# google-research/multinerf

Measured on AMD Instinct MI355X. Metric: train_rays_per_sec, higher is better.
Workload: dtype bf16 MFMA inputs / fp32 accumulate, fp32 everywhere else

## Files before the change

### include/mnerf.h

```cpp
#ifndef MNERF_H_
#define MNERF_H_

#include <stdint.h>

#ifdef __cplusplus
extern "C" {
#endif

typedef enum {
  MNR_OK = 0,
  MNR_ERR_INVALID_ARGUMENT = -1,
  MNR_ERR_HIP = -2,
  MNR_ERR_UNSUPPORTED = -3
} mnr_status;

const char* mnr_last_error(void);
int mnr_abi_version(void);
int mnr_device_info(int device, int* cu_count, int* lds_bytes_per_cu, char* arch_name, int arch_name_len);

typedef enum { MNR_RAYDIST_IDENTITY = 0, MNR_RAYDIST_RECIPROCAL = 1, MNR_RAYDIST_PIECEWISE = 2,
               MNR_RAYDIST_LOG = 3, MNR_RAYDIST_EXP = 4, MNR_RAYDIST_SQRT = 5, MNR_RAYDIST_SQUARE = 6 } mnr_raydist;

typedef struct {
  int n_prev;
// ... 201 lines not shown
  float density_noise_std;
  int has_rgb;
  int rgb_act;
  float rgb_premultiplier, rgb_bias, rgb_padding;
  int bg_mode;
  float bg_value;
} mnr_composite_cfg;

int mnr_composite_fwd(const mnr_composite_cfg* cfg, int64_t B, const float* raw_density,
                      const float* density_noise, const float* raw_rgb, const float* tdist,
                      const float* dirs, const float* bg, const float* exposure_scale,
                      float* density, float* rgb, float* weights, float* rgb_out, float* acc,
                      void* stream);

int mnr_composite_bwd(const mnr_composite_cfg* cfg, int64_t B, const float* raw_density,
                      const float* density_noise, const float* raw_rgb, const float* tdist,
                      const float* dirs, const float* bg, const float* exposure_scale,
                      const float* weights, const float* g_rgb_out, const float* g_weights,
                      float* g_raw_density, uint16_t* g_raw_density_bf16, int ld_bf16,
                      float* g_raw_rgb, float* g_exposure_scale , void* stream);

typedef struct {
  mnr_composite_cfg cfg;
  int64_t B, B_valid;
  const float* raw_density; const float* density_noise; const float* raw_rgb; const float* tdist; const float* dirs;
  const float* bg; const float* exposure_scale; const float* weights;
  const float* g_rgb_out;
  const float* g_weights;
  float* g_raw_density; uint16_t* g_raw_density_bf16; int ld_bf16; float* g_raw_rgb; float* g_exposure_scale;
  int data_loss_type; float charb_padding; float data_loss_mult;
  const float* rgb_out; const float* gt; const float* lossmult; int lm_c; const float* denom; float* data_stats;
  int wloss_mode; float wloss_mult; const float* sdist; int n_ref; const float* t_ref; const float* w_ref; float* wloss_stat;
  float* g_x;
} mnr_level_bwd_args;
int mnr_level_bwd(const mnr_level_bwd_args* args, void* stream);

typedef struct {
  int64_t B, B_valid; int n;
  const float* sdist; const float* near; const float* far; int raydist_fn;
  const float* g_x; const float* raw_density; const float* density_noise; float density_noise_std; float density_bias;
  int density_act; const float* dirs;
  const float* g_t0; const float* g_t1;
  float distortion_mult; const float* weights;
  const float* g_sdist_in;
  float* g_sdist;
} mnr_sdist_bwd_args;
int mnr_sdist_bwd(const mnr_sdist_bwd_args* args, void* stream);

int mnr_exposure_scale(int64_t B, const float* exposure_values, const int32_t* exposure_idx,
                       const float* offsets, float* out, void* stream);
int mnr_exposure_scale_bwd(int64_t B_valid, const float* exposure_values, const int32_t* exposure_idx,
                           const float* g_scale, float* g_offsets, void* stream);

int mnr_render_extras(int64_t B, int n, const float* weights, const float* tdist, const float* t_far,
                      float* out, void* stream);

typedef struct {
  int T; int lmax;
  const int32_t* m; const int32_t* l;
  const float* sigma;
  const float* mat;
} mnr_ide_tables;

#define MNR_REF_PRED_NORMALS    1
#define MNR_REF_DENSITY_NORMALS 2
#define MNR_REF_REFLECT         4
// ... 385 lines not shown
```

### include/mnerf_debug.h

```cpp
#ifndef MNERF_DEBUG_H_
#define MNERF_DEBUG_H_

#ifdef __cplusplus
extern "C" {
#endif

int mnr_debug_gemm_timeline(unsigned long long* device_buffer);
int mnr_gemm_nt_set_pipelined(int on);
int mnr_gemm_nt_set_persistent(int wgs_per_cu);
int mnr_gemm_nt_set_wres(int max_wgs);
int mnr_gemm_nt_panel_set_max_wgs(int n);

int mnr_mlp_chain_set_deferred(int on);

int mnr_mlp_chain_set_max_wgs(int n);

int mnr_debug_chain_timeline(unsigned long long* device_buffer);

int mnr_level_bwd_set_quad(int on);

#ifdef __cplusplus
}
#endif
#endif
```

### multinerf_amd/_lib.py

```python

import ctypes as C
import os
import re

HERE = os.path.dirname(os.path.abspath(__file__))
LIB_PATH = os.environ.get('MNR_LIB_PATH') or os.path.join(HERE, 'libmnerf_hip.so')
LIB_F32_PATH = os.path.join(HERE, 'libmnerf_hip_f32.so')
HEADER_PATH = os.path.join(os.path.dirname(HERE), 'include', 'mnerf.h')
F32_ABSENT = ('mnr_mlp_chain_fwd', 'mnr_mlp_chain_fwd_ipe', 'mnr_mlp_chain_bwd')


def describe():
  stamp = LIB_PATH + '.stamp'
  digest = None
  if os.path.exists(stamp):
    with open(stamp) as f:
      digest = f.read().strip()
  return {'path': os.path.relpath(LIB_PATH, os.path.dirname(HERE)), 'overridden': bool(os.environ.get('MNR_LIB_PATH')),
          'source_digest': digest, 'extra_hipcc_flags': os.environ.get('MNR_EXTRA_HIPCC_FLAGS', '')}

MNR_OK = 0
MNR_ERR_INVALID_ARGUMENT = -1

RAYDIST = {None: 0, 'identity': 0, 'reciprocal': 1, 'piecewise': 2, 'log': 3, 'exp': 4, 'sqrt': 5,
# ... 63 lines not shown
  _fields_ = [('cfg', IpeCfg), ('n', C.c_int), ('tdist', vp), ('origins', vp), ('directions', vp), ('radii', vp),
              ('basis', vp)]


class MlpChainBwdArgs(C.Structure):
  _fields_ = [('M', C.c_int64), ('W', C.c_int), ('depth', C.c_int),
              ('g_head', vp), ('w_head', vp),
              ('bits', vp * CHAIN_MAX_DEPTH), ('Bw', vp * CHAIN_MAX_DEPTH), ('ldb', C.c_int * CHAIN_MAX_DEPTH),
              ('dY', vp * CHAIN_MAX_DEPTH), ('dY_in', vp)]


class PackDesc(C.Structure):
  _fields_ = [('src_off', C.c_int64), ('rows_in', C.c_int), ('cols_out', C.c_int),
              ('dst_off', C.c_int64), ('ld', C.c_int), ('row0', C.c_int), ('col0', C.c_int),
              ('transpose', C.c_int)]


class CompositeCfg(C.Structure):
  _fields_ = [('n', C.c_int), ('opaque_background', C.c_int), ('density_act', C.c_int),
              ('density_bias', C.c_float), ('density_noise_std', C.c_float), ('has_rgb', C.c_int),
              ('rgb_act', C.c_int), ('rgb_premultiplier', C.c_float), ('rgb_bias', C.c_float),
              ('rgb_padding', C.c_float), ('bg_mode', C.c_int), ('bg_value', C.c_float)]


class LevelBwdArgs(C.Structure):
  _fields_ = [('cfg', CompositeCfg), ('B', C.c_int64), ('B_valid', C.c_int64),
              ('raw_density', vp), ('density_noise', vp), ('raw_rgb', vp), ('tdist', vp), ('dirs', vp),
              ('bg', vp), ('exposure_scale', vp), ('weights', vp), ('g_rgb_out', vp), ('g_weights', vp),
              ('g_raw_density', vp), ('g_raw_density_bf16', vp), ('ld_bf16', C.c_int), ('g_raw_rgb', vp),
              ('g_exposure_scale', vp),
              ('data_loss_type', C.c_int), ('charb_padding', C.c_float), ('data_loss_mult', C.c_float),
              ('rgb_out', vp), ('gt', vp), ('lossmult', vp), ('lm_c', C.c_int), ('denom', vp), ('data_stats', vp),
              ('wloss_mode', C.c_int), ('wloss_mult', C.c_float), ('sdist', vp), ('n_ref', C.c_int), ('t_ref', vp),
              ('w_ref', vp), ('wloss_stat', vp), ('g_x', vp)]


class SdistBwdArgs(C.Structure):
  _fields_ = [('B', C.c_int64), ('B_valid', C.c_int64), ('n', C.c_int),
              ('sdist', vp), ('near', vp), ('far', vp), ('raydist_fn', C.c_int),
              ('g_x', vp), ('raw_density', vp), ('density_noise', vp), ('density_noise_std', C.c_float),
              ('density_bias', C.c_float), ('density_act', C.c_int), ('dirs', vp),
              ('g_t0', vp), ('g_t1', vp), ('distortion_mult', C.c_float), ('weights', vp),
              ('g_sdist_in', vp), ('g_sdist', vp)]


class IdeTables(C.Structure):
  _fields_ = [('T', C.c_int), ('lmax', C.c_int), ('m', vp), ('l', vp), ('sigma', vp), ('mat', vp)]


class RobustArgs(C.Structure):
  _fields_ = [('B', C.c_int64), ('B_valid', C.c_int64),
              ('patch_size', C.c_int), ('inner_patch_size', C.c_int), ('filter_size', C.c_int), ('enable', C.c_int),
              ('smoothed_inlier_quantile', C.c_double), ('inner_patch_inlier_quantile', C.c_double),
              ('rgb', vp), ('gt', vp), ('lossmult', vp), ('lm_c', C.c_int), ('loss_threshold', vp), ('denom', vp),
              ('mask', vp), ('lossmult_out', vp), ('err', vp), ('stats', vp), ('mse', vp)]


SSIM_MAX_FILTER = 11
CC_FEATURES, CC_GRAM_OUT = 10, 65


class SsimArgs(C.Structure):
  _fields_ = [('H', C.c_int), ('W', C.c_int), ('C', C.c_int), ('crop', C.c_int), ('filter_size', C.c_int),
              ('filter_sigma', C.c_double), ('max_val', C.c_double), ('k1', C.c_double), ('k2', C.c_double),
              ('a', vp), ('b', vp), ('map', vp), ('partials', vp), ('out', vp)]


# ... 207 lines not shown
    'mnr_atlas_uvs': ([C.POINTER(AtlasArgs), vp, vp], i32),
    'mnr_raster_visibility': ([C.POINTER(RasterArgs), vp, vp, vp, vp], i32),
    'mnr_raster_shade': ([C.POINTER(RasterArgs), vp, vp, vp, vp, vp, vp, vp, vp], i32),
    'mnr_shtex_weights': ([vp, i64, vp, i64, vp, vp], i32),
    'mnr_shtex_fit': ([vp, vp, i64, i32, vp, vp, i64, C.c_double, vp, vp], i32),
    'mnr_shtex_shade': ([C.POINTER(ShtexShadeArgs), vp, vp], i32),
    'mnr_mesh_grid_count': ([C.POINTER(MeshDistArgs), vp, vp], i32),
    'mnr_mesh_grid_fill': ([C.POINTER(MeshDistArgs), vp, i64, vp, vp, vp], i32),
    'mnr_mesh_distance': ([C.POINTER(MeshDistArgs), vp, vp, i64, vp, vp, i64, f32, vp, vp, vp, vp], i32),
    'mnr_mesh_face_areas': ([vp, i64, vp, i64, vp, vp], i32),
    'mnr_mesh_sample': ([vp, i64, vp, i64, vp, i64, C.c_uint32, vp, vp, vp], i32),
    'mnr_mesh_closest': ([vp, i64, vp, i64, vp, vp, vp, i64, vp, vp, vp], i32),
    'mnr_mesh_face_normals': ([vp, i64, vp, i64, vp, vp], i32),
    'mnr_icp_sums_partials': ([i64], i32),
    'mnr_icp_sums': ([i64, vp, vp, vp, vp, C.POINTER(C.c_double), vp, vp, vp], i32),
    'mnr_crop_polygon': ([vp, i64, vp, i32, i32, C.c_double, C.c_double, vp, vp], i32),
    'mnr_mesh_raycast': ([C.POINTER(MeshDistArgs), vp, vp, i64, vp, vp, vp, i64, f32, f32, i32, vp, vp, vp, vp], i32),
    'mnr_raycast_shade': ([C.POINTER(RasterArgs), vp, vp, i64, vp, vp, vp], i32),
    'mnr_weight_decay': ([vp, i64, i64, f32, vp, vp, vp, vp], i32),
    'mnr_grad_sqnorm': ([vp, i64, i64, f32, vp, vp], i32),
    'mnr_clip_adam': ([C.POINTER(AdamCfg), i64, i64, vp, vp, vp, vp, vp, vp], i32),
}

_DEBUG_PROTOS = {
    'mnr_debug_gemm_timeline': ([vp], i32),
    'mnr_gemm_nt_set_persistent': ([i32], i32),
    'mnr_level_bwd_set_quad': ([i32], i32),
    'mnr_gemm_nt_set_pipelined': ([i32], i32),
    'mnr_gemm_nt_set_wres': ([i32], i32),
    'mnr_gemm_nt_panel_set_max_wgs': ([i32], i32),
    'mnr_debug_chain_timeline': ([vp], i32),
    'mnr_mlp_chain_set_deferred': ([i32], i32),
    'mnr_mlp_chain_set_max_wgs': ([i32], i32),
}

_lib = None


def header_symbols(path=None):
  with open(path or HEADER_PATH) as f:
    text = f.read()
  text = re.sub(r'/\*.*?\*/', '', text, flags=re.S)
  return sorted(set(re.findall(r'\b(mnr_[a-z0-9_]+)\s*\(', text)))


def _bind(path, absent=()):
  if not os.path.exists(path):
    raise RuntimeError(
        f'{path} is missing: the HIP extension has not been built. Run '
        '`python -m multinerf_amd.build` (needs hipcc, ROCm >= 7.0). There is no CPU fallback.')
  import torch
  lib = C.CDLL(path)
  lib.mnr_last_error.restype = C.c_char_p
  lib.mnr_last_error.argtypes = []
  for name, (argtypes, restype) in _PROTOS.items():
    if name in absent:
      continue
    fn = getattr(lib, name)
    fn.argtypes = argtypes
    fn.restype = restype
  return lib


_lib_f32 = None
_f32_depth = 0

# ... 54 lines not shown
```

### multinerf_amd/csrc/gemm.hip

```cpp
#include <stdio.h>
#include <stdlib.h>
#include <type_traits>

#include "common.h"

#ifdef MNR_DENSE_F32
#include "dense_f32.inc"
#else


#define NT_CPAD 16

template <int MI_, int NJ_, int WM_, int WN_, int EPI_BATCH_ = 0, int BIAS_LDS_ = 0, int PIPE_ = 0, int DBG_ = 0, int BK_ = 64, int STAGES_ = 2>
struct NtCfg {
  static constexpr int DBG = DBG_;
  static constexpr bool PIPE = PIPE_ != 0;
  static constexpr int EPI_BATCH = EPI_BATCH_;
  static constexpr int MI = MI_, NJ = NJ_, WM = WM_, WN = WN_, BK = BK_, STAGES = STAGES_;
  static constexpr int MINW = 1;
  static constexpr int BM = 32 * MI * WM, BN = 32 * NJ * WN;
  static constexpr int THREADS = 64 * WM * WN;
  static constexpr int ROWB = BK * 2;
  static constexpr int SLOTS = ROWB / 16;
  static constexpr int A_BYTES = BM * ROWB, B_BYTES = BN * ROWB;
// ... 540 lines not shown
  if (rl < row_lanes) {
    for (int64_t r = r0 + rl; r < r1; r += row_lanes) {
      const bf16x8 v = *(const bf16x8*)(X + r * ld + cg * 8);
#pragma unroll
      for (int e = 0; e < 8; ++e) s[e] += (float)v[e];
    }
  }
#pragma unroll
  for (int e = 0; e < 8; ++e) red[threadIdx.x * 8 + e] = s[e];
  __syncthreads();
  if (rl == 0) {
    for (int k = 1; k < row_lanes; ++k)
#pragma unroll
      for (int e = 0; e < 8; ++e) s[e] += red[(k * lanes_per_row + cg) * 8 + e];
#pragma unroll
    for (int e = 0; e < 8; ++e)
      if (cg * 8 + e < n_valid) unsafeAtomicAdd(out + cg * 8 + e, s[e]);
  }
}

extern "C" int mnr_colsum_bf16(const uint16_t* X, int ld, int64_t M, int n_valid, float* out, void* stream) {
  MNR_CHECK_ARG(X && out && M > 0 && n_valid > 0, "mnr_colsum_bf16: bad arguments");
  MNR_CHECK_ARG(ld % 8 == 0 && (n_valid + 7) / 8 <= 256 && ((n_valid + 7) / 8) * 8 <= ld,
                "mnr_colsum_bf16: need ld %% 8 == 0 and n_valid <= min(ld, 2048)");
  const int rows_per_block = 1024;
  const int grid = mnr_cdiv(M, rows_per_block);
  hipLaunchKernelGGL(colsum_kernel, dim3(grid), dim3(256), 0, (hipStream_t)stream, (const bf16*)X, ld, M,
                     n_valid, rows_per_block, out);
  MNR_CHECK_LAUNCH();
  return MNR_OK;
}


__global__ void pack_weights_kernel(const float* __restrict__ params, const mnr_pack_desc* __restrict__ descs,
                                    bf16* __restrict__ dst) {
  const mnr_pack_desc d = descs[blockIdx.y];
  const int total = d.rows_in * d.cols_out;
  for (int e = blockIdx.x * blockDim.x + threadIdx.x; e < total; e += gridDim.x * blockDim.x) {
    int r, c;
    if (d.transpose) {
      c = e / d.rows_in;
      r = e % d.rows_in;
    } else {
      r = e / d.cols_out;
      c = e % d.cols_out;
    }
    const float v = params[d.src_off + (int64_t)r * d.cols_out + c];
    const int64_t o = d.transpose ? d.dst_off + (int64_t)(d.row0 + c) * d.ld + d.col0 + r
                                  : d.dst_off + (int64_t)(d.row0 + r) * d.ld + d.col0 + c;
    dst[o] = (bf16)v;
  }
}

extern "C" int mnr_pack_weights_bf16(const float* params, const mnr_pack_desc* descs_device, int n_desc,
                                     int max_elems, uint16_t* dst, void* stream) {
  MNR_CHECK_ARG(params && descs_device && dst && n_desc > 0 && max_elems > 0, "mnr_pack_weights_bf16: bad arguments");
  int gx = mnr_cdiv(max_elems, 256);
  if (gx > 64) gx = 64;
  hipLaunchKernelGGL(pack_weights_kernel, dim3(gx, n_desc), dim3(256), 0, (hipStream_t)stream, params,
                     descs_device, (bf16*)dst);
  MNR_CHECK_LAUNCH();
  return MNR_OK;
}

__global__ void scatter_add_kernel(const float* __restrict__ src, int ld_src, int row0, int col0, int rows,
                                   int cols, float* __restrict__ dst, int ld_dst) {
  const int total = rows * cols;
  for (int e = blockIdx.x * blockDim.x + threadIdx.x; e < total; e += gridDim.x * blockDim.x) {
    const int k = e / cols, c = e % cols;
    dst[(int64_t)k * ld_dst + c] += src[(int64_t)(row0 + k) * ld_src + col0 + c];
  }
}

extern "C" int mnr_scatter_add_f32(const float* src, int ld_src, int row0, int col0, int rows, int cols,
                                   float* dst, int ld_dst, void* stream) {
  MNR_CHECK_ARG(src && dst && rows > 0 && cols > 0, "mnr_scatter_add_f32: bad arguments");
  int grid = mnr_cdiv((long long)rows * cols, 256);
  if (grid > 2048) grid = 2048;
  hipLaunchKernelGGL(scatter_add_kernel, dim3(grid), dim3(256), 0, (hipStream_t)stream, src, ld_src, row0,
                     col0, rows, cols, dst, ld_dst);
  MNR_CHECK_LAUNCH();
  return MNR_OK;
}

__global__ void cast_f32_bf16_kernel(const float* __restrict__ src, int ld_src, int64_t M, int n,
                                     bf16* __restrict__ dst, int ld_dst, int col0) {
  const int64_t total = M * n;
  for (int64_t e = (int64_t)blockIdx.x * blockDim.x + threadIdx.x; e < total; e += (int64_t)gridDim.x * blockDim.x) {
    const int64_t r = e / n;
    const int c = (int)(e % n);
    dst[r * ld_dst + col0 + c] = (bf16)src[r * ld_src + c];
// ... 299 lines not shown
```

### multinerf_amd/csrc/render.hip

```cpp
#include "common.h"
#include "ray_losses.h"

#define CP_THREADS 64

__device__ __forceinline__ float cp_act(int kind, float x) {
  switch (kind) {
    case MNR_ACT_SIGMOID: return mnr_sigmoid(x);
    case MNR_ACT_SAFE_EXP: return expf(fminf(x, 88.0f));
    case MNR_ACT_SOFTPLUS: return mnr_softplus(x);
    case MNR_ACT_EXP: return expf(x);
    case MNR_ACT_RELU: return fmaxf(x, 0.0f);
    default: return x;
  }
}

__device__ __forceinline__ float cp_act_grad(int kind, float x, float y) {
  switch (kind) {
    case MNR_ACT_SIGMOID: return y * (1.0f - y);
    case MNR_ACT_SAFE_EXP: return y;
    case MNR_ACT_SOFTPLUS: return mnr_sigmoid(x);
    case MNR_ACT_EXP: return y;
    case MNR_ACT_RELU: return x > 0.0f ? 1.0f : 0.0f;
    default: return 1.0f;
  }
// ... 440 lines not shown
        carry += Lanes<LPR>::suffix_total(inc);
        if (in) {
          float gx = ghat * l_tn[i] - after;
          if (c.opaque_background && i == n - 1) gx = 0.0f;
          l_den[i] = gx * l_dg[i];
          l_gh[i] = gx;
        }
      }
    }
    if (a.g_exposure_scale) {
#pragma unroll
      for (int ch = 0; ch < 3; ++ch) {
        const float g = Lanes<LPR>::sum(ges[ch]);
        if (live && q == 0) a.g_exposure_scale[ray * 3 + ch] += g;
      }
    }
  }
  if (a.data_loss_type >= 0 && a.data_stats) {
    s_mse = ls_wave_sum(s_mse);
    s_dloss = ls_wave_sum(s_dloss);
    if (threadIdx.x == 0) {
      const float denom = *a.denom;
      unsafeAtomicAdd(a.data_stats + 0, s_mse / denom);
      unsafeAtomicAdd(a.data_stats + 1, a.data_loss_mult * s_dloss / denom);
    }
  }
  if (a.wloss_mode != 0 && a.wloss_stat) {
    s_wloss = ls_wave_sum(s_wloss);
    const float norm = a.wloss_mode == 1 ? (float)a.B_valid * (float)a.n_ref : (float)a.B_valid;
    if (threadIdx.x == 0) unsafeAtomicAdd(a.wloss_stat, a.wloss_mult * s_wloss / norm);
  }
  __syncthreads();
  if (a.g_raw_density) cp_rows_out(lds, L.stride, L.den, a.g_raw_density + ray0 * n, rows, n);
  if (a.g_raw_density_bf16) {
    bf16* gb = (bf16*)a.g_raw_density_bf16;
    for (int e = threadIdx.x; e < rows * n; e += CP_THREADS) {
      const int rr = e / n, i = e - rr * n;
      gb[(ray0 * n + e) * (int64_t)a.ld_bf16] = (bf16)lds[rr * L.stride + L.den + i];
    }
  }
  if (c.has_rgb && a.g_raw_rgb) cp_rows_out(lds, L.stride, L.rgb, a.g_raw_rgb + ray0 * n * 3, rows, 3 * n);
  if (a.g_x) cp_rows_out(lds, L.stride, L.scr + 2 * n, a.g_x + ray0 * n, rows, n);
}

template <int LPR>
static void level_bwd_launch(const CpPlan& p, const mnr_level_bwd_args* a, void* stream) {
  static unsigned long long attr_set = 0;
  if (p.lds > 64 * 1024 && mnr_attr_needed(&attr_set))
    (void)hipFuncSetAttribute((const void*)level_bwd_kernel<LPR>, hipFuncAttributeMaxDynamicSharedMemorySize, 160 * 1024);
  hipLaunchKernelGGL(level_bwd_kernel<LPR>, dim3(mnr_cdiv(a->B, p.rays)), dim3(CP_THREADS), p.lds, (hipStream_t)stream, *a, p.rays);
}

extern "C" int mnr_level_bwd(const mnr_level_bwd_args* a, void* stream) {
  MNR_CHECK_ARG(a != nullptr, "mnr_level_bwd: null args");
  const mnr_composite_cfg* cfg = &a->cfg;
  MNR_CHECK_ARG(a->B > 0 && a->B_valid > 0 && a->B_valid <= a->B && a->raw_density && a->tdist && a->dirs && a->weights,
                "mnr_level_bwd: null argument");
  MNR_CHECK_ARG(cfg->n >= 1 && cfg->n <= 1024, "mnr_level_bwd: n out of range");
  MNR_CHECK_ARG(a->g_raw_density || a->g_raw_density_bf16, "mnr_level_bwd: no density-gradient output");
  MNR_CHECK_ARG(!cfg->has_rgb || a->raw_rgb, "mnr_level_bwd: has_rgb needs raw_rgb");
  MNR_CHECK_ARG(cfg->bg_mode == 0 || a->bg, "mnr_level_bwd: bg_mode 1 needs bg");
  MNR_CHECK_ARG(a->data_loss_type < 0 || (a->data_loss_type <= MNR_LOSS_RAWNERF && a->rgb_out && a->gt && a->lossmult &&
                                          a->denom && (a->lm_c == 1 || a->lm_c == 3)),
                "mnr_level_bwd: the fused data loss needs rgb_out, gt, lossmult [B,1|3] and denom");
  MNR_CHECK_ARG(a->wloss_mode >= 0 && a->wloss_mode <= 2, "mnr_level_bwd: wloss_mode must be 0, 1 or 2");
  MNR_CHECK_ARG(a->wloss_mode == 0 || a->sdist, "mnr_level_bwd: weight losses need this level's sdist");
  MNR_CHECK_ARG(a->wloss_mode != 1 || (a->n_ref >= 1 && a->n_ref <= 1024 && a->t_ref && a->w_ref),
                "mnr_level_bwd: the interlevel loss needs the final level's (t_ref, w_ref)");
  const CpPlan p = cp_plan(cfg->n, cfg->has_rgb, true, a->wloss_mode, a->n_ref, a->B);
  MNR_CHECK_ARG(p.lds <= 160 * 1024, "mnr_level_bwd: n=%d too long for LDS staging", cfg->n);
  (p.lpr == 4 ? level_bwd_launch<4> : level_bwd_launch<1>)(p, a, stream);
// ... 233 lines not shown
```

### multinerf_amd/csrc/resample.hip

```cpp
#include "common.h"

#pragma clang fp contract(off)

#define RS_THREADS 64

__device__ __forceinline__ float rs_s_to_t(int fn, float s, float near, float far) {
  float fn_near, fn_far;
  switch (fn) {
    case MNR_RAYDIST_RECIPROCAL: fn_near = 1.0f / near; fn_far = 1.0f / far; break;
    case MNR_RAYDIST_PIECEWISE:
      fn_near = near < 1.0f ? 0.5f * near : 1.0f - 0.5f / near;
      fn_far = far < 1.0f ? 0.5f * far : 1.0f - 0.5f / far;
      break;
    case MNR_RAYDIST_LOG: fn_near = logf(near); fn_far = logf(far); break;
    case MNR_RAYDIST_EXP: fn_near = expf(near); fn_far = expf(far); break;
    case MNR_RAYDIST_SQRT: fn_near = sqrtf(near); fn_far = sqrtf(far); break;
    case MNR_RAYDIST_SQUARE: fn_near = near * near; fn_far = far * far; break;
    default: fn_near = near; fn_far = far; break;
  }
  const float x = s * fn_far + (1.0f - s) * fn_near;
  switch (fn) {
    case MNR_RAYDIST_RECIPROCAL: return 1.0f / x;
    case MNR_RAYDIST_PIECEWISE: return x < 0.5f ? 2.0f * x : 0.5f / (1.0f - x);
    case MNR_RAYDIST_LOG: return expf(x);
// ... 251 lines not shown
  for (int j = j0; j < j1; ++j) {
    float u = u_base[j];
    if (jitter) u = u + (c.single_jitter ? jit1 : jitter[ray * n + j] * c.max_jitter);
    if (cur == -2) {
      int lo_i = -1, hi_i = nb + 1;
      while (hi_i - lo_i > 1) {
        const int mid = (lo_i + hi_i) >> 1;
        if (cw[mid] <= u) lo_i = mid;
        else hi_i = mid;
      }
      cur = lo_i;
    }
    centers[j] = rs_interp_one(u, cw, td, 1, nb + 1, cur);
    if (idx_out && g < nrays) idx_out[ray * n + j] = cur;
  }
  __syncthreads();
  float* so = base + lay.SO;
  for (int j = l; j <= n; j += RSP_LPR) {
    float v;
    if (j == 0) v = fmaxf(c.domain_lo, 2.0f * centers[0] - (centers[1] + centers[0]) / 2.0f);
    else if (j == n) v = fminf(c.domain_hi, 2.0f * centers[n - 1] - (centers[n - 1] + centers[n - 2]) / 2.0f);
    else v = (centers[j] + centers[j - 1]) / 2.0f;
    so[j] = v;
  }
  __syncthreads();
  for (int e = threadIdx.x; e < nrays * (n + 1); e += RS_THREADS) {
    const int rr = e / (n + 1), i = e % (n + 1);
    const float sv = lds[rr * lay.per_ray + lay.SO + i];
    sdist_out[ray0 * (n + 1) + e] = sv;
    tdist_out[ray0 * (n + 1) + e] = rs_s_to_t(c.raydist_fn, sv, near[ray0 + rr], far[ray0 + rr]);
  }
}

static RspLay rsp_layout(int np, int n) {
  RspLay l;
  const int m = 3 * np + 1;
  int o = 0;
  l.T = o; o += np + 1;
  l.P = o; o += np;
  l.TD = o; o += m;
  l.WD = o; o += m;
  l.CW = o; o += m;
  l.CEN = o; o += n;
  l.SO = o; o += n + 1;
  l.RED = o; o += RSP_LPR;
  l.per_ray = (o + 3) & ~3;
  return l;
}

extern "C" int mnr_resample_level(const mnr_resample_cfg* cfg, int64_t B, const float* sdist_prev,
                                  const float* w_prev, const float* u_base, const float* jitter,
                                  const float* near, const float* far, float* sdist_out, float* tdist_out,
                                  int32_t* idx_out, void* stream) {
  MNR_CHECK_ARG(cfg && B > 0 && sdist_prev && w_prev && u_base && near && far && sdist_out && tdist_out,
                "mnr_resample_level: null argument");
  MNR_CHECK_ARG(cfg->n_samples > 1, "num_samples must be > 1, is %d.", cfg->n_samples);
  MNR_CHECK_ARG(cfg->n_prev >= 1 && cfg->n_prev <= 1024 && cfg->n_samples <= 1024,
                "mnr_resample_level: n_prev=%d / n_samples=%d out of range", cfg->n_prev, cfg->n_samples);
  MNR_CHECK_ARG(cfg->raydist_fn >= 0 && cfg->raydist_fn <= MNR_RAYDIST_SQUARE, "mnr_resample_level: bad raydist_fn");
  const RspLay lay = rsp_layout(cfg->n_prev, cfg->n_samples);
  const size_t lds_bytes = (size_t)lay.per_ray * RSP_RPW * 4;
  MNR_CHECK_ARG(lds_bytes <= 160 * 1024, "mnr_resample_level: step function too long for LDS");
  static unsigned long long attr_set = 0;
  if (mnr_attr_needed(&attr_set)) {
    (void)hipFuncSetAttribute((const void*)resample_level_kernel, hipFuncAttributeMaxDynamicSharedMemorySize,
                              160 * 1024);
  }
  const int grid = mnr_cdiv(B, RSP_RPW);
  hipLaunchKernelGGL(resample_level_kernel, dim3(grid), dim3(RS_THREADS), lds_bytes, (hipStream_t)stream, *cfg,
                     B, lay, sdist_prev, w_prev, u_base, jitter, near, far, sdist_out, tdist_out, idx_out);
  MNR_CHECK_LAUNCH();
  return MNR_OK;
}


__global__ void sorted_interp_kernel(int64_t B, int nc, int nu, const float* u, const float* cw, const float* t,
                                     float* out, int32_t* idx) {
  const int64_t b = (int64_t)blockIdx.x * blockDim.x + threadIdx.x;
  if (b >= B) return;
  int cur = -1;
  for (int j = 0; j < nu; ++j) {
    out[b * nu + j] = rs_interp_one(u[b * nu + j], cw + b * nc, t + b * nc, 1, nc, cur);
    if (idx) idx[b * nu + j] = cur;
  }
}

extern "C" int mnr_sorted_interp(int64_t B, int nc, int nu, const float* u, const float* cw, const float* t,
                                 float* out, int32_t* idx, void* stream) {
  MNR_CHECK_ARG(B > 0 && nc > 0 && nu > 0 && u && cw && t && out, "mnr_sorted_interp: bad arguments");
  hipLaunchKernelGGL(sorted_interp_kernel, dim3(mnr_cdiv(B, 64)), dim3(64), 0, (hipStream_t)stream, B, nc, nu, u,
                     cw, t, out, idx);
  MNR_CHECK_LAUNCH();
// ... 412 lines not shown
```

### multinerf_amd/models.py

```python

import ctypes as C
import dataclasses
import math
from typing import Any, Dict, List, Optional, Tuple

import numpy as np
import torch

from multinerf_amd import _lib as L
from multinerf_amd import geopoly
from multinerf_amd import gin
from multinerf_amd import ops
from multinerf_amd import utils

F32_EPS = float(np.finfo(np.float32).eps)
bf16 = torch.bfloat16
f32 = torch.float32


def _rup(x, m):
  return (x + m - 1) // m * m


def _in_library(fn):
# ... 1395 lines not shown
                             exposure_scale=expo, g_exposure_scale=g_expo if expo is not None else None, losses=losses,
                             g_x_out=g_x_out, **kw)

  def _density_head_bwd(self, b: _LevelBwd, g_raw_density, dA):
    plan, M, W, d = b.plan, b.M, b.plan.W, b.plan.density
    ops.small_head_bwd(b.mlp['acts'][-1], W, g_raw_density.view(M, 1), b.flat[d.kernel_off:d.kernel_off + W].view(W, 1), M=M, K=W, Cn=1,
                       dX=dA, lddx=0 if dA is None else W, relu_mask=b.relu and dA is not None,
                       dW=b.gslice(d.kernel_off, W), db=b.gslice(d.bias_off, 1))
    if dA is not None:
      b.act_vjp(b.mlp['zs'][-1] if not b.relu else None, dA)

  def _head4_bwd(self, b: _LevelBwd, g_raw_density, g_rgb, dA):
    plan, M, W, flat = b.plan, b.M, b.plan.W, b.flat
    g4 = self._buf(('bwd', b.slot, 'g4'), (M, 4), f32)
    g4[:, 0].copy_(g_raw_density.view(M))
    g4[:, 1:4].copy_(g_rgb.view(M, 3))
    dn, dr = plan.density, plan.rgb
    w4 = self._buf(('bwd', b.slot, 'w4', W), (W, 4), f32)
    w4[:, 0].copy_(flat[dn.kernel_off:dn.kernel_off + W])
    w4[:, 1:4].copy_(flat[dr.kernel_off:dr.kernel_off + 3 * W].view(W, 3))
    t4 = self._buf(('bwd', b.slot, 't4', W), (W + 1, 4), f32)
    t4.zero_()
    ops.small_head_bwd(b.mlp['acts'][-1], W, g4, w4, M=M, K=W, Cn=4, dX=dA, lddx=W, relu_mask=b.relu, dW=t4[:W].view(-1), db=t4[W])
    b.act_vjp(b.mlp['zs'][-1] if not b.relu else None, dA)
    for (d, c0) in plan.head_segs:
      ops.scatter_add(t4, 4, 0, c0, W, d.fan_out, b.gslice(d.kernel_off, W * d.fan_out), d.fan_out)
      ops.scatter_add(t4, 4, W, c0, 1, d.fan_out, b.gslice(d.bias_off, d.fan_out), d.fan_out)

  def _merged_head_composite_vjp(self, b: _LevelBwd, g_rgb_out, g_weights, g_expo, losses, g_x_out):
    plan, M, route = b.plan, b.M, b.route
    bw, nh = plan.hp.bottleneck_width, plan.packed['head']['nb_pad']
    dHB = self._buf(('bwd', b.slot, 'dHB', nh, plan.module_name), (M, nh), bf16, zero=True)
    assert route.gcol or not route.panel
    g_den_f32, g_rgb = self._composite_vjp(b.lv, g_rgb_out, g_weights, g_expo, losses, g_x_out, g_den_bf16=dHB.view(-1)[bw:],
                                           ld_bf16=nh, want_f32=route.gcol)
    g_vec = None
    if route.gcol:
      g_vec = self._buf(('bwd', b.slot, 'g_den_vec'), (M,), bf16)
      ops.cast_f32_to_bf16(g_den_f32.view(-1), 1, M, 1, g_vec, 1, 0)
      ops.colsum(dHB.view(-1)[bw:], M, 1, b.gslice(plan.density.bias_off, 1), ld=nh)
    return dHB, g_vec, g_rgb.view(M, 3)

  def _color_bwd(self, b: _LevelBwd, g_raw_rgb, dHB):
    plan, mlp, flat, M, n, relu, gslice = b.plan, b.mlp, b.flat, b.M, b.n, b.relu, b.gslice
    hp, bw, nh, slot = plan.hp, plan.hp.bottleneck_width, dHB.shape[1], b.slot
    if plan.diffuse_on:
      g_raw_rgb = ops.ref_color_bwd(mlp['raw_rgb_pre'], mlp['small'], hp.rgb_premultiplier, hp.rgb_bias, hp.rgb_padding,
                                    hp.use_specular_tint, g_raw_rgb.contiguous(), dHB, bw + 4, bw + 7)
    WV, NV, VI, vacts, d = hp.net_width_viewdirs, len(plan.view), mlp['VI'], mlp['vacts'], plan.rgb
    dy = b.dv_buf(NV - 1, NV)
    ops.small_head_bwd(vacts[-1], WV, g_raw_rgb, flat[d.kernel_off:d.kernel_off + d.fan_in * 3].view(d.fan_in, 3), M=M, K=WV, Cn=3,
                       dX=dy, lddx=WV, relu_mask=relu, dW=gslice(d.kernel_off, d.fan_in * 3), db=gslice(d.bias_off, 3))
    b.act_vjp(mlp['vzs'][-1] if not relu else None, dy)
    dVIa = dVIb = None
    want_glo = plan.glo > 0 and self._glo_cam is not None
    gGa = self._buf(('bwd', slot, 'gGa'), (M, plan.glo), f32) if want_glo else None
    gGb = None
    glo_kw = lambda t: dict(Cf=t, ldcf=plan.glo, f0=plan.glo_col, nf=plan.glo) if want_glo else {}
    for i in reversed(range(len(plan.view))):
      d, concat = plan.view[i]
      e = plan.packed[('view', i)]
      inp = VI if i == 0 else vacts[i - 1]
      in_w = plan.ldVI if i == 0 else WV
      ops.gemm_tn(inp, dy, gslice(d.kernel_off, d.fan_in * d.fan_out), M=M, K=in_w, N=WV, lda=inp.stride(0), ldb=WV, ldc=d.fan_out,
                  k_valid=(plan.vi_width if i == 0 else WV), n_valid=d.fan_out, bias_out=gslice(d.bias_off, d.fan_out),
                  bias_n_valid=d.fan_out)
      if concat:
        ops.gemm_tn(VI, dy, gslice(d.kernel_off + WV * d.fan_out, plan.vi_width * d.fan_out), M=M, K=plan.ldVI, N=WV, lda=plan.ldVI,
                    ldb=WV, ldc=d.fan_out, k_valid=plan.vi_width, n_valid=d.fan_out)
        first_skip = dVIb is None
        tVI = self._buf(('bwd', slot, 'dVIb', 0 if first_skip else 1), (M, plan.ldVI), bf16)
        tG = self._buf(('bwd', slot, 'gGb', 0 if first_skip else 1), (M, plan.glo), f32) if want_glo else None
        B2 = self._w(plan, e['b2_off'], plan.ldVI, e['b_ld'])
# ... 256 lines not shown
```

### multinerf_amd/ops.py

```python

import ctypes as C
import math
import os

import torch

from multinerf_amd import _lib as L

bf16 = torch.bfloat16
f32 = torch.float32


def _ptr(t):
  return None if t is None else C.c_void_p(t.data_ptr())


def _stream():
  return C.c_void_p(torch.cuda.current_stream().cuda_stream)


def _on_device(t):
  return t.is_cuda


# ... 659 lines not shown

def composite_cfg(n, *, opaque_background, density_act, density_bias, density_noise_std, has_rgb, rgb_act,
                  rgb_premultiplier, rgb_bias, rgb_padding, bg_mode, bg_value):
  return L.CompositeCfg(n, int(opaque_background), L.ACT[density_act], float(density_bias),
                        float(density_noise_std), int(has_rgb), L.ACT[rgb_act], float(rgb_premultiplier),
                        float(rgb_bias), float(rgb_padding), int(bg_mode), float(bg_value))


def composite_fwd(cfg, raw_density, tdist, dirs, *, raw_rgb=None, density_noise=None, bg=None,
                  exposure_scale=None, want_acc=True):
  _chk(raw_density, f32, 'raw_density')
  _chk(tdist, f32, 'tdist')
  _chk(dirs, f32, 'dirs')
  for x, nm in ((raw_rgb, 'raw_rgb'), (density_noise, 'density_noise'), (bg, 'bg'),
                (exposure_scale, 'exposure_scale')):
    _chk(x, f32, nm, allow_none=True)
  B, n = raw_density.shape
  dev = raw_density.device
  density = torch.empty((B, n), dtype=f32, device=dev)
  weights = torch.empty((B, n), dtype=f32, device=dev)
  rgb = torch.empty((B, n, 3), dtype=f32, device=dev) if cfg.has_rgb else None
  rgb_out = torch.empty((B, 3), dtype=f32, device=dev)
  acc = torch.empty((B,), dtype=f32, device=dev) if want_acc else None
  _e = PROFILE.start()
  L.check(lib().mnr_composite_fwd(C.byref(cfg), B, _ptr(raw_density), _ptr(density_noise), _ptr(raw_rgb),
                                  _ptr(tdist), _ptr(dirs), _ptr(bg), _ptr(exposure_scale), _ptr(density),
                                  _ptr(rgb), _ptr(weights), _ptr(rgb_out), _ptr(acc), _stream()))
  PROFILE.stop(_e, 'composite_fwd', 4 * (raw_density.numel() * (2 + 2 + (6 if raw_rgb is not None else 0))))
  return density, rgb, weights, rgb_out, acc


def composite_bwd(cfg, raw_density, tdist, dirs, weights, *, raw_rgb=None, density_noise=None, bg=None,
                  exposure_scale=None, g_rgb_out=None, g_weights=None, g_den_bf16=None, ld_bf16=0,
                  want_f32=True, g_exposure_scale=None, losses=None, g_raw_density_out=None, g_x_out=None):
  B, n = raw_density.shape
  dev = raw_density.device
  for x, nm in ((raw_density, 'raw_density'), (tdist, 'tdist'), (dirs, 'dirs'), (weights, 'weights')):
    _chk(x, f32, nm)
  for x, nm in ((g_rgb_out, 'g_rgb_out'), (g_weights, 'g_weights')):
    _chk(x, f32, nm, allow_none=True)
  _chk(g_den_bf16, bf16, 'g_den_bf16', allow_none=True)
  if g_raw_density_out is not None:
    _chk(g_raw_density_out, f32, 'g_raw_density_out')
    assert want_f32 and g_raw_density_out.shape == (B, n) and g_raw_density_out.is_contiguous()
    g_raw_density = g_raw_density_out
  else:
    g_raw_density = torch.empty((B, n), dtype=f32, device=dev) if want_f32 else None
  g_raw_rgb = torch.empty((B, n, 3), dtype=f32, device=dev) if cfg.has_rgb else None
  a = L.LevelBwdArgs()
  a.cfg = cfg
  a.B = B
  a.B_valid = B if losses is None else int(losses['B_valid'])
  p = lambda t: None if t is None else t.data_ptr()
  a.raw_density, a.density_noise, a.raw_rgb, a.tdist, a.dirs = p(raw_density), p(density_noise), p(raw_rgb), p(tdist), p(dirs)
  a.bg, a.exposure_scale, a.weights, a.g_rgb_out, a.g_weights = p(bg), p(exposure_scale), p(weights), p(g_rgb_out), p(g_weights)
  a.g_raw_density, a.g_raw_density_bf16, a.ld_bf16 = p(g_raw_density), p(g_den_bf16), ld_bf16
  a.g_raw_rgb, a.g_exposure_scale = p(g_raw_rgb), p(g_exposure_scale)
  a.data_loss_type, a.wloss_mode = -1, 0
  if g_x_out is not None:
    _chk(g_x_out, f32, 'g_x_out')
    assert g_x_out.shape == (B, n) and g_x_out.is_contiguous()
    a.g_x = p(g_x_out)
  keep = []
  if losses is not None and losses.get('data') is not None:
    d = losses['data']
    if d['type'] not in L.DATA_LOSS:
      raise ValueError(f"unsupported data_loss_type {d['type']!r}")
    for k in ('rgb_out', 'gt', 'lossmult', 'denom', 'stats'):
      _chk(d[k], f32, 'data.' + k)
    assert d['rgb_out'].shape[0] == B and d['gt'].shape[0] == B and d['lossmult'].shape[0] == B
    a.data_loss_type, a.charb_padding, a.data_loss_mult = L.DATA_LOSS[d['type']], float(d['charb_padding']), float(d['mult'])
    a.rgb_out, a.gt, a.lossmult, a.lm_c = p(d['rgb_out']), p(d['gt']), p(d['lossmult']), d['lossmult'].shape[-1]
    a.denom, a.data_stats = p(d['denom']), p(d['stats'])
    keep.append(d)
  if losses is not None and losses.get('weights') is not None:
    w = losses['weights']
    _chk(w['sdist'], f32, 'weights.sdist')
    _chk(w['stat'], f32, 'weights.stat')
    assert w['sdist'].shape == (B, n + 1)
    a.wloss_mult, a.sdist, a.wloss_stat = float(w['mult']), p(w['sdist']), p(w['stat'])
    if w['mode'] == 'interlevel':
      _chk(w['t_ref'], f32, 'weights.t_ref')
      _chk(w['w_ref'], f32, 'weights.w_ref')
      assert w['t_ref'].shape[0] == B and w['t_ref'].shape[1] == w['w_ref'].shape[1] + 1
      a.wloss_mode, a.n_ref, a.t_ref, a.w_ref = 1, w['w_ref'].shape[1], p(w['t_ref']), p(w['w_ref'])
    elif w['mode'] == 'distortion':
      a.wloss_mode = 2
    else:
      raise ValueError(f"weights.mode {w['mode']!r}")
    keep.append(w)
  _e = PROFILE.start()
  L.check(lib().mnr_level_bwd(C.byref(a), _stream()))
  PROFILE.stop(_e, 'composite_bwd', 4 * (raw_density.numel() * (3 + (3 if raw_rgb is not None else 0))) + (2 + (12 if raw_rgb is not None else 0)) * raw_density.numel())
  return g_raw_density, g_raw_rgb

# ... 1422 lines not shown
```

Measured before the change: 534,800.

## Fuse density-grad cast and bias colsum into composite bwd; specialize resample; tile weight packing

The composite backward kernel now writes the bf16 density-gradient vector directly and accumulates the density bias gradient with a wave reduction plus atomic add. This removes a separate f32 write, a cast kernel and a colsum kernel. A templated resample kernel for n_prev=64 with 64 or 32 output samples uses fixed-unroll binary searches in place of the generic layout path. Weight packing now transposes through a 64x64 LDS tile with vectorized loads and stores. The atomic bias accumulation makes the result order-dependent and relies on the bias slot being zeroed beforehand.

```diff
diff --git a/include/mnerf.h b/include/mnerf.h
--- a/include/mnerf.h
+++ b/include/mnerf.h
@@ -257,6 +257,7 @@
   const float* rgb_out; const float* gt; const float* lossmult; int lm_c; const float* denom; float* data_stats;
   int wloss_mode; float wloss_mult; const float* sdist; int n_ref; const float* t_ref; const float* w_ref; float* wloss_stat;
   float* g_x;
+  uint16_t* g_vec; float* db_density;
 } mnr_level_bwd_args;
 int mnr_level_bwd(const mnr_level_bwd_args* args, void* stream);
 
diff --git a/include/mnerf_debug.h b/include/mnerf_debug.h
--- a/include/mnerf_debug.h
+++ b/include/mnerf_debug.h
@@ -19,6 +19,8 @@
 
 int mnr_level_bwd_set_quad(int on);
 
+int mnr_resample_set_generic(int on);
+
 #ifdef __cplusplus
 }
 #endif
diff --git a/multinerf_amd/_lib.py b/multinerf_amd/_lib.py
--- a/multinerf_amd/_lib.py
+++ b/multinerf_amd/_lib.py
@@ -119,7 +119,7 @@
               ('data_loss_type', C.c_int), ('charb_padding', C.c_float), ('data_loss_mult', C.c_float),
               ('rgb_out', vp), ('gt', vp), ('lossmult', vp), ('lm_c', C.c_int), ('denom', vp), ('data_stats', vp),
               ('wloss_mode', C.c_int), ('wloss_mult', C.c_float), ('sdist', vp), ('n_ref', C.c_int), ('t_ref', vp),
-              ('w_ref', vp), ('wloss_stat', vp), ('g_x', vp)]
+              ('w_ref', vp), ('wloss_stat', vp), ('g_x', vp), ('g_vec', vp), ('db_density', vp)]
 
 
 class SdistBwdArgs(C.Structure):
@@ -393,6 +393,7 @@
     'mnr_debug_chain_timeline': ([vp], i32),
     'mnr_mlp_chain_set_deferred': ([i32], i32),
     'mnr_mlp_chain_set_max_wgs': ([i32], i32),
+    'mnr_resample_set_generic': ([i32], i32),
 }
 
 _lib = None
diff --git a/multinerf_amd/csrc/gemm.hip b/multinerf_amd/csrc/gemm.hip
--- a/multinerf_amd/csrc/gemm.hip
+++ b/multinerf_amd/csrc/gemm.hip
@@ -596,31 +596,86 @@
 }
 
 
-__global__ void pack_weights_kernel(const float* __restrict__ params, const mnr_pack_desc* __restrict__ descs,
-                                    bf16* __restrict__ dst) {
+#define PK_TILE 64
+
+__global__ __launch_bounds__(256) void pack_weights_kernel(const float* __restrict__ params,
+                                                           const mnr_pack_desc* __restrict__ descs, bf16* __restrict__ dst) {
+  __shared__ float tile[PK_TILE][PK_TILE + 1];
   const mnr_pack_desc d = descs[blockIdx.y];
-  const int total = d.rows_in * d.cols_out;
-  for (int e = blockIdx.x * blockDim.x + threadIdx.x; e < total; e += gridDim.x * blockDim.x) {
-    int r, c;
-    if (d.transpose) {
-      c = e / d.rows_in;
-      r = e % d.rows_in;
+  const int tiles_c = (d.cols_out + PK_TILE - 1) / PK_TILE;
+  const int n_tiles = ((d.rows_in + PK_TILE - 1) / PK_TILE) * tiles_c;
+  const float* src = params + d.src_off;
+  bf16* out = dst + d.dst_off + (int64_t)d.row0 * d.ld + d.col0;
+  const bool vec_src = ((d.src_off | (int64_t)d.cols_out) & 3) == 0 && ((uintptr_t)params & 15) == 0;
+  const bool vec_dst = ((d.dst_off | (int64_t)d.ld | (int64_t)d.col0) & 3) == 0 && ((uintptr_t)dst % sizeof(bf16x4)) == 0;
+  const int g4 = (threadIdx.x & 15) * 4;
+  const int h = threadIdx.x >> 4;
+  for (int tix = blockIdx.x; tix < n_tiles; tix += gridDim.x) {
+    const int ti = tix / tiles_c;
+    const int r0 = ti * PK_TILE, c0 = (tix - ti * tiles_c) * PK_TILE;
+#pragma unroll
+    for (int p = 0; p < PK_TILE / 16; ++p) {
+      const int lr = h + 16 * p, r = r0 + lr, c = c0 + g4;
+      if (r < d.rows_in) {
+        const float* s = src + (int64_t)r * d.cols_out + c;
+        if (vec_src && c + 3 < d.cols_out) {
+          const f32x4 v = *(const f32x4*)s;
+#pragma unroll
+          for (int k = 0; k < 4; ++k) tile[lr][g4 + k] = v[k];
+        } else {
+#pragma unroll
+          for (int k = 0; k < 4; ++k)
+            if (c + k < d.cols_out) tile[lr][g4 + k] = s[k];
+        }
+      }
+    }
+    __syncthreads();
+    if (!d.transpose) {
+#pragma unroll
+      for (int p = 0; p < PK_TILE / 16; ++p) {
+        const int lr = h + 16 * p, r = r0 + lr, c = c0 + g4;
+        if (r < d.rows_in) {
+          bf16* o = out + (int64_t)r * d.ld + c;
+          if (vec_dst && c + 3 < d.cols_out) {
+            bf16x4 v;
+#pragma unroll
+            for (int k = 0; k < 4; ++k) v[k] = (bf16)tile[lr][g4 + k];
+            *(bf16x4*)o = v;
+          } else {
+#pragma unroll
+            for (int k = 0; k < 4; ++k)
+              if (c + k < d.cols_out) o[k] = (bf16)tile[lr][g4 + k];
+          }
+        }
+      }
     } else {
-      r = e / d.cols_out;
-      c = e % d.cols_out;
-    }
-    const float v = params[d.src_off + (int64_t)r * d.cols_out + c];
-    const int64_t o = d.transpose ? d.dst_off + (int64_t)(d.row0 + c) * d.ld + d.col0 + r
-                                  : d.dst_off + (int64_t)(d.row0 + r) * d.ld + d.col0 + c;
-    dst[o] = (bf16)v;
+#pragma unroll
+      for (int p = 0; p < PK_TILE / 16; ++p) {
+        const int lc = h + 16 * p, c = c0 + lc, r = r0 + g4;
+        if (c < d.cols_out) {
+          bf16* o = out + (int64_t)c * d.ld + r;
+          if (vec_dst && r + 3 < d.rows_in) {
+            bf16x4 v;
+#pragma unroll
+            for (int k = 0; k < 4; ++k) v[k] = (bf16)tile[g4 + k][lc];
+            *(bf16x4*)o = v;
+          } else {
+#pragma unroll
+            for (int k = 0; k < 4; ++k)
+              if (r + k < d.rows_in) o[k] = (bf16)tile[g4 + k][lc];
+          }
+        }
+      }
+    }
+    __syncthreads();
   }
 }
 
 extern "C" int mnr_pack_weights_bf16(const float* params, const mnr_pack_desc* descs_device, int n_desc,
                                      int max_elems, uint16_t* dst, void* stream) {
   MNR_CHECK_ARG(params && descs_device && dst && n_desc > 0 && max_elems > 0, "mnr_pack_weights_bf16: bad arguments");
-  int gx = mnr_cdiv(max_elems, 256);
-  if (gx > 64) gx = 64;
+  int gx = mnr_cdiv(max_elems, PK_TILE * PK_TILE);
+  if (gx > 65535) gx = 65535;
   hipLaunchKernelGGL(pack_weights_kernel, dim3(gx, n_desc), dim3(256), 0, (hipStream_t)stream, params,
                      descs_device, (bf16*)dst);
   MNR_CHECK_LAUNCH();
diff --git a/multinerf_amd/csrc/render.hip b/multinerf_amd/csrc/render.hip
--- a/multinerf_amd/csrc/render.hip
+++ b/multinerf_amd/csrc/render.hip
@@ -496,11 +496,20 @@
   }
   __syncthreads();
   if (a.g_raw_density) cp_rows_out(lds, L.stride, L.den, a.g_raw_density + ray0 * n, rows, n);
-  if (a.g_raw_density_bf16) {
+  if (a.g_raw_density_bf16 || a.g_vec || a.db_density) {
     bf16* gb = (bf16*)a.g_raw_density_bf16;
+    bf16* gv = (bf16*)a.g_vec;
+    float s_db = 0.0f;
     for (int e = threadIdx.x; e < rows * n; e += CP_THREADS) {
       const int rr = e / n, i = e - rr * n;
-      gb[(ray0 * n + e) * (int64_t)a.ld_bf16] = (bf16)lds[rr * L.stride + L.den + i];
+      const bf16 hv = (bf16)lds[rr * L.stride + L.den + i];
+      if (gb) gb[(ray0 * n + e) * (int64_t)a.ld_bf16] = hv;
+      if (gv) gv[ray0 * n + e] = hv;
+      s_db += (float)hv;
+    }
+    if (a.db_density) {
+      s_db = ls_wave_sum(s_db);
+      if (threadIdx.x == 0) unsafeAtomicAdd(a.db_density, s_db);
     }
   }
   if (c.has_rgb && a.g_raw_rgb) cp_rows_out(lds, L.stride, L.rgb, a.g_raw_rgb + ray0 * n * 3, rows, 3 * n);
diff --git a/multinerf_amd/csrc/resample.hip b/multinerf_amd/csrc/resample.hip
--- a/multinerf_amd/csrc/resample.hip
+++ b/multinerf_amd/csrc/resample.hip
@@ -307,6 +307,225 @@
   }
 }
 
+template <int NP, int N>
+struct RspS {
+  static constexpr int M = 3 * NP + 1;
+  static constexpr int NW = M - 1;
+  static constexpr int NB = 3 * NP - 2;
+  static constexpr int CHW = NW / RSP_LPR;
+  static constexpr int CH = (NB + RSP_LPR - 1) / RSP_LPR;
+  static constexpr int CHS = N / RSP_LPR;
+  static constexpr int T = 0, P = NP + 1;
+  static constexpr int CEN = 0, SO = N;
+  static constexpr int TD = 2 * NP + 1;
+  static constexpr int WD = TD + M;
+  static constexpr int CW = WD;
+  static constexpr int RED = WD + M;
+  static constexpr int PER_RAY = (RED + RSP_LPR + 3) & ~3;
+  static_assert(NW % RSP_LPR == 0 && N % RSP_LPR == 0 && 2 * N + 1 <= TD && NP + 1 <= 127, "shape outside the specialisation");
+};
+
+__device__ __forceinline__ int rsp_count_fixed(const float* a, int n, float shift, float x, bool le) {
+  int pos = 0;
+#pragma unroll
+  for (int s = 64; s >= 1; s >>= 1) {
+    const int nxt = pos + s;
+    const float v = a[min(nxt, n) - 1] + shift;
+    const bool take = nxt <= n && (le ? (v <= x) : (v < x));
+    pos = take ? nxt : pos;
+  }
+  return pos;
+}
+
+template <int NP, int N>
+__global__ __launch_bounds__(RS_THREADS) void resample_level_special_kernel(
+    mnr_resample_cfg c, int64_t B, const float* __restrict__ sdist_prev, const float* __restrict__ w_prev,
+    const float* __restrict__ u_base, const float* __restrict__ jitter, const float* __restrict__ near,
+    const float* __restrict__ far, float* __restrict__ sdist_out, float* __restrict__ tdist_out,
+    int32_t* __restrict__ idx_out) {
+  typedef RspS<NP, N> S;
+  __shared__ __attribute__((aligned(16))) float lds[RSP_RPW * S::PER_RAY];
+  const int64_t ray0 = (int64_t)blockIdx.x * RSP_RPW;
+  const int nrays = (int)min((int64_t)RSP_RPW, B - ray0);
+  for (int e = threadIdx.x; e < RSP_RPW * (NP + 1); e += RS_THREADS) {
+    const int r = e / (NP + 1), i = e % (NP + 1);
+    lds[r * S::PER_RAY + S::T + i] = sdist_prev[(ray0 + min(r, nrays - 1)) * (NP + 1) + i];
+  }
+  for (int e = threadIdx.x; e < RSP_RPW * NP; e += RS_THREADS) {
+    const int r = e / NP, i = e % NP;
+    lds[r * S::PER_RAY + S::P + i] = w_prev[(ray0 + min(r, nrays - 1)) * NP + i];
+  }
+  const int g = threadIdx.x / RSP_LPR, l = threadIdx.x % RSP_LPR;
+  const int gr = min(g, nrays - 1);
+  __syncthreads();
+  float* base = lds + g * S::PER_RAY;
+  const float* t = base + S::T;
+  float* p = base + S::P;
+  float* tdf = base + S::TD;
+  float* wdf = base + S::WD;
+  float* red = base + S::RED;
+  const float eps2 = MNR_F32_EPS * MNR_F32_EPS;
+  const float dil = c.dilation;
+
+#pragma unroll
+  for (int i = 0; i < NP / RSP_LPR; ++i) {
+    const int j = l + RSP_LPR * i;
+    p[j] = p[j] / fmaxf(eps2, t[j + 1] - t[j]);
+  }
+#pragma unroll
+  for (int i = 0; i < (S::M + RSP_LPR - 1) / RSP_LPR; ++i) {
+    const int e_raw = l + RSP_LPR * i;
+    const int e = min(e_raw, S::M - 1);
+    const bool isa = e <= NP, isc = e > 2 * NP;
+    const int own = isa ? e : (isc ? e - (2 * NP + 1) : e - (NP + 1));
+    const float tv = t[isc ? own + 1 : own];
+    const float v = isa ? tv : (isc ? tv + dil : tv - dil);
+    const int c1 = rsp_count_fixed(t, isa ? NP : NP + 1, isa ? -dil : 0.0f, v, !(!isa && !isc));
+    const int c2 = rsp_count_fixed(isc ? t : t + 1, NP, isc ? -dil : dil, v, isc);
+    if (e_raw < S::M) tdf[own + c1 + c2] = fminf(fmaxf(v, c.domain_lo), c.domain_hi);
+  }
+  __syncthreads();
+  {
+    const int k0 = l * S::CHW;
+    float wv[S::CHW];
+    float csum = 0.0f;
+    int jhi = rsp_count_fixed(t, NP, -dil, tdf[k0], true) - 1;
+    int jlo = rsp_count_fixed(t + 1, NP, dil, tdf[k0], true);
+#pragma unroll
+    for (int i = 0; i < S::CHW; ++i) {
+      const int k = k0 + i;
+      const float x = tdf[k];
+      while (jhi + 1 < NP && t[jhi + 1] - dil <= x) ++jhi;
+      while (jlo < NP && !(t[jlo + 1] + dil > x)) ++jlo;
+      float best = 0.0f;
+      for (int j = jlo; j <= jhi; ++j) best = fmaxf(best, p[j]);
+      wv[i] = best * (tdf[k + 1] - x);
+      csum += wv[i];
+    }
+    float total;
+    (void)rsp_chunk_offset(csum, red, l, total);
+    const float denom = fmaxf(eps2, total);
+#pragma unroll
+    for (int i = 0; i < S::CHW; ++i) wdf[k0 + i] = wv[i] / denom;
+    __syncthreads();
+  }
+
+  const float* td = tdf + 1;
+  const int k0 = l * S::CH;
+  float tdv[S::CH + 1], wv[S::CH];
+#pragma unroll
+  for (int i = 0; i <= S::CH; ++i) tdv[i] = td[min(k0 + i, S::NB)];
+#pragma unroll
+  for (int i = 0; i < S::CH; ++i) wv[i] = wdf[1 + min(k0 + i, S::NB - 1)];
+  float mx = -INFINITY;
+#pragma unroll
+  for (int i = 0; i < S::CH; ++i) {
+    const bool open = tdv[i + 1] > tdv[i];
+    const float lg = open ? c.anneal * rs_log(wv[i] + c.resample_padding) : -INFINITY;
+    wv[i] = lg;
+    if (k0 + i < S::NB) mx = (lg != lg || mx != mx) ? NAN : fmaxf(mx, lg);
+  }
+  __syncthreads();
+  red[l] = mx;
+  __syncthreads();
+  mx = -INFINITY;
+#pragma unroll
+  for (int i = 0; i < RSP_LPR; ++i) {
+    const float v = red[i];
+    mx = (v != v || mx != mx) ? NAN : fmaxf(mx, v);
+  }
+  float csum = 0.0f;
+#pragma unroll
+  for (int i = 0; i < S::CH; ++i) {
+    const float e = rs_exp(wv[i] - mx);
+    wv[i] = e;
+    if (k0 + i < S::NB) csum += e;
+  }
+  float denom;
+  (void)rsp_chunk_offset(csum, red, l, denom);
+  csum = 0.0f;
+#pragma unroll
+  for (int i = 0; i < S::CH; ++i) {
+    const float wk = wv[i] / denom;
+    wv[i] = wk;
+    if (k0 + i < S::NB - 1) csum += wk;
+  }
+  float unused;
+  const float off = rsp_chunk_offset(csum, red, l, unused);
+  float* cw = base + S::CW;
+  float run = 0.0f;
+#pragma unroll
+  for (int i = 0; i < S::CH; ++i) {
+    if (k0 + i < S::NB - 1) {
+      run += wv[i];
+      const float cs = off + run;
+      cw[k0 + i + 1] = (cs != cs) ? cs : fminf(1.0f, cs);
+    }
+  }
+  if (l == 0) {
+    cw[0] = 0.0f;
+    cw[S::NB] = 1.0f;
+  }
+  __syncthreads();
+
+  float* centers = base + S::CEN;
+  const int64_t ray = ray0 + gr;
+  const int j0 = l * S::CHS;
+  const float jit1 = (jitter && c.single_jitter) ? jitter[ray] * c.max_jitter : 0.0f;
+  int cur = -2;
+#pragma unroll
+  for (int i = 0; i < S::CHS; ++i) {
+    const int j = j0 + i;
+    float u = u_base[j];
+    if (jitter) u = u + (c.single_jitter ? jit1 : jitter[ray * N + j] * c.max_jitter);
+    if (i == 0) {
+      int lo_i = -1, hi_i = S::NB + 1;
+      while (hi_i - lo_i > 1) {
+        const int mid = (lo_i + hi_i) >> 1;
+        if (cw[mid] <= u) lo_i = mid;
+        else hi_i = mid;
+      }
+      cur = lo_i;
+    }
+    centers[j] = rs_interp_one(u, cw, td, 1, S::NB + 1, cur);
+    if (idx_out && g < nrays) idx_out[ray * N + j] = cur;
+  }
+  __syncthreads();
+  float* so = base + S::SO;
+#pragma unroll
+  for (int i = 0; i < (N + RSP_LPR) / RSP_LPR; ++i) {
+    const int j = l + RSP_LPR * i;
+    if (j <= N) {
+      float v;
+      if (j == 0) v = fmaxf(c.domain_lo, 2.0f * centers[0] - (centers[1] + centers[0]) / 2.0f);
+      else if (j == N) v = fminf(c.domain_hi, 2.0f * centers[N - 1] - (centers[N - 1] + centers[N - 2]) / 2.0f);
+      else v = (centers[j] + centers[j - 1]) / 2.0f;
+      so[j] = v;
+    }
+  }
+  __syncthreads();
+  for (int e = threadIdx.x; e < nrays * (N + 1); e += RS_THREADS) {
+    const int rr = e / (N + 1), i = e % (N + 1);
+    const float sv = lds[rr * S::PER_RAY + S::SO + i];
+    sdist_out[ray0 * (N + 1) + e] = sv;
+    tdist_out[ray0 * (N + 1) + e] = rs_s_to_t(c.raydist_fn, sv, near[ray0 + rr], far[ray0 + rr]);
+  }
+}
+
+static int g_rs_generic = 0;
+extern "C" int mnr_resample_set_generic(int on) {
+  g_rs_generic = on != 0;
+  return MNR_OK;
+}
+
+template <int NP, int N>
+static void rsp_launch_special(const mnr_resample_cfg* cfg, int64_t B, const float* sdist_prev, const float* w_prev,
+                               const float* u_base, const float* jitter, const float* near, const float* far,
+                               float* sdist_out, float* tdist_out, int32_t* idx_out, void* stream) {
+  hipLaunchKernelGGL((resample_level_special_kernel<NP, N>), dim3(mnr_cdiv(B, RSP_RPW)), dim3(RS_THREADS), 0,
+                     (hipStream_t)stream, *cfg, B, sdist_prev, w_prev, u_base, jitter, near, far, sdist_out, tdist_out, idx_out);
+}
+
 static RspLay rsp_layout(int np, int n) {
   RspLay l;
   const int m = 3 * np + 1;
@@ -333,6 +552,12 @@
   MNR_CHECK_ARG(cfg->n_prev >= 1 && cfg->n_prev <= 1024 && cfg->n_samples <= 1024,
                 "mnr_resample_level: n_prev=%d / n_samples=%d out of range", cfg->n_prev, cfg->n_samples);
   MNR_CHECK_ARG(cfg->raydist_fn >= 0 && cfg->raydist_fn <= MNR_RAYDIST_SQUARE, "mnr_resample_level: bad raydist_fn");
+  if (!g_rs_generic && cfg->use_dilation && cfg->n_prev == 64 && (cfg->n_samples == 64 || cfg->n_samples == 32)) {
+    (cfg->n_samples == 64 ? rsp_launch_special<64, 64> : rsp_launch_special<64, 32>)(
+        cfg, B, sdist_prev, w_prev, u_base, jitter, near, far, sdist_out, tdist_out, idx_out, stream);
+    MNR_CHECK_LAUNCH();
+    return MNR_OK;
+  }
   const RspLay lay = rsp_layout(cfg->n_prev, cfg->n_samples);
   const size_t lds_bytes = (size_t)lay.per_ray * RSP_RPW * 4;
   MNR_CHECK_ARG(lds_bytes <= 160 * 1024, "mnr_resample_level: step function too long for LDS");
diff --git a/multinerf_amd/models.py b/multinerf_amd/models.py
--- a/multinerf_amd/models.py
+++ b/multinerf_amd/models.py
@@ -1451,13 +1451,10 @@
     bw, nh = plan.hp.bottleneck_width, plan.packed['head']['nb_pad']
     dHB = self._buf(('bwd', b.slot, 'dHB', nh, plan.module_name), (M, nh), bf16, zero=True)
     assert route.gcol or not route.panel
-    g_den_f32, g_rgb = self._composite_vjp(b.lv, g_rgb_out, g_weights, g_expo, losses, g_x_out, g_den_bf16=dHB.view(-1)[bw:],
-                                           ld_bf16=nh, want_f32=route.gcol)
-    g_vec = None
-    if route.gcol:
-      g_vec = self._buf(('bwd', b.slot, 'g_den_vec'), (M,), bf16)
-      ops.cast_f32_to_bf16(g_den_f32.view(-1), 1, M, 1, g_vec, 1, 0)
-      ops.colsum(dHB.view(-1)[bw:], M, 1, b.gslice(plan.density.bias_off, 1), ld=nh)
+    g_vec = self._buf(('bwd', b.slot, 'g_den_vec'), (M,), bf16) if route.gcol else None
+    _, g_rgb = self._composite_vjp(b.lv, g_rgb_out, g_weights, g_expo, losses, g_x_out, g_den_bf16=dHB.view(-1)[bw:],
+                                   ld_bf16=nh, want_f32=False, g_vec_out=g_vec,
+                                   db_density=b.gslice(plan.density.bias_off, 1) if route.gcol else None)
     return dHB, g_vec, g_rgb.view(M, 3)
 
   def _color_bwd(self, b: _LevelBwd, g_raw_rgb, dHB):
diff --git a/multinerf_amd/ops.py b/multinerf_amd/ops.py
--- a/multinerf_amd/ops.py
+++ b/multinerf_amd/ops.py
@@ -715,7 +715,8 @@
 
 def composite_bwd(cfg, raw_density, tdist, dirs, weights, *, raw_rgb=None, density_noise=None, bg=None,
                   exposure_scale=None, g_rgb_out=None, g_weights=None, g_den_bf16=None, ld_bf16=0,
-                  want_f32=True, g_exposure_scale=None, losses=None, g_raw_density_out=None, g_x_out=None):
+                  want_f32=True, g_exposure_scale=None, losses=None, g_raw_density_out=None, g_x_out=None,
+                  g_vec_out=None, db_density=None):
   B, n = raw_density.shape
   dev = raw_density.device
   for x, nm in ((raw_density, 'raw_density'), (tdist, 'tdist'), (dirs, 'dirs'), (weights, 'weights')):
@@ -744,6 +745,14 @@
     _chk(g_x_out, f32, 'g_x_out')
     assert g_x_out.shape == (B, n) and g_x_out.is_contiguous()
     a.g_x = p(g_x_out)
+  if g_vec_out is not None:
+    _chk(g_vec_out, bf16, 'g_vec_out')
+    assert g_vec_out.numel() == B * n and g_vec_out.is_contiguous()
+    a.g_vec = p(g_vec_out)
+  if db_density is not None:
+    _chk(db_density, f32, 'db_density')
+    assert db_density.numel() == 1
+    a.db_density = p(db_density)
   keep = []
   if losses is not None and losses.get('data') is not None:
     d = losses['data']
```

New measurement: 538,200 (median of 6 runs). No clear change (+0.6%).
